# DaehwanKimLab/centrifuge

Hardware: NVIDIA H100
Metric: reads/sec (100 bp SE classification) (higher is better)
Workload: dtype u64

## Files before the change

### centrifuge_b200/capi.py

```python
import ctypes as C
import os

import numpy as np

HERE = os.path.dirname(os.path.abspath(__file__))
LIB_PATH = os.path.join(HERE, "libcfb200.so")

CFB_UID_NONE = 0xFFFFFFFF
REC_DTYPE = np.dtype([("taxid", "<u8"), ("score", "<u4"), ("hitlen", "<u4"), ("uid", "<u4"), ("pad", "<u4")])

_lib = None


class CfbError(RuntimeError):
    pass


class IndexInfo(C.Structure):
    _fields_ = [("len", C.c_uint64), ("num_sides", C.c_uint64), ("n_seqs", C.c_uint64), ("n_tax_nodes", C.c_uint64),
                ("n_boundaries", C.c_uint64), ("line_rate", C.c_int32), ("off_rate", C.c_int32), ("ftab_chars", C.c_int32),
                ("sample_bytes", C.c_int32), ("compressed", C.c_int32), ("device", C.c_int32), ("device_bytes", C.c_uint64)]


class IndexTables(C.Structure):
# ... 267 lines not shown
        out = np.zeros(3 * n, dtype=np.uint64)
        _ck(lib().cfb_counts_dense(self.h, C.c_int(1 if global_ else 0), _p(out, C.c_uint64), C.c_uint64(out.size)))
        return out.reshape(3, n)

    def comm_init_rank(self, nranks, rank, uid):
        buf = (C.c_uint8 * 128).from_buffer_copy(bytes(uid))
        _ck(lib().cfb_comm_init_rank(self.h, C.c_int(nranks), C.c_int(rank), buf))

    def counts_allreduce(self, out=None):
        arr = (C.c_void_p * 1)(self.h)
        _ck(lib().cfb_counts_allreduce(arr, C.c_int(1), _p(out, C.c_uint64) if out is not None else None, C.c_uint64(out.size if out is not None else 0)))

    def requests(self):
        out = (C.c_uint64 * 5)()
        _ck(lib().cfb_ctx_requests(self.h, out))
        return dict(zip(["rank16", "ftab2", "ftabk", "walk8", "ftabd"], [int(x) for x in out]))

    def request_breakdown(self):
        out = (C.c_uint64 * 8)()
        _ck(lib().cfb_ctx_request_breakdown(self.h, out))
        names = ["rank16_w1", "rank16_w2_4", "rank16_w5", "walk8_try_row", "walk8_ok_row", "walk8_try_range", "walk8_ok_range", "walk8_ok_w5"]
        return dict(zip(names, [int(x) for x in out]))

    def counters(self):
        out = (C.c_uint64 * 8)()
        _ck(lib().cfb_ctx_counters(self.h, out))
        names = ["units", "partial_searches", "ftab_probes", "sides_search", "walk_steps", "rows_resolved", "lf_steps", "ext_searches"]
        return dict(zip(names, [int(x) for x in out]))

    def launches(self):
        n = C.c_uint64()
        _ck(lib().cfb_ctx_kernel_launches(self.h, C.byref(n)))
        return int(n.value)

    def close(self):
        if self.h:
            lib().cfb_ctx_destroy(self.h)
            self.h = C.c_void_p()


def comm_unique_id():
    buf = (C.c_uint8 * 128)()
    _ck(lib().cfb_comm_unique_id(buf))
    return bytes(buf)


def comm_init_all(contexts):
    arr = (C.c_void_p * len(contexts))(*[c.h for c in contexts])
    _ck(lib().cfb_comm_init_all(arr, C.c_int(len(contexts))))


def counts_allreduce_all(contexts):
    arr = (C.c_void_p * len(contexts))(*[c.h for c in contexts])
    _ck(lib().cfb_counts_allreduce(arr, C.c_int(len(contexts)), None, C.c_uint64(0)))


def gather_ceiling(index, table, n_requests=1 << 30):
    g, ms = C.c_double(), C.c_double()
    _ck(lib().cfb_gather_ceiling(index.h, C.c_int(table), C.c_uint64(n_requests), C.byref(g), C.byref(ms)))
    return float(g.value), float(ms.value)


def test_lf(index, rows, chars):
    rows = np.ascontiguousarray(rows, dtype=np.uint64)
    chars = np.ascontiguousarray(chars, dtype=np.uint8)
    out = np.zeros(len(rows), dtype=np.uint64)
    _ck(lib().cfb_test_lf(index.h, _p(rows, C.c_uint64), _p(chars, C.c_uint8), C.c_uint64(len(rows)), _p(out, C.c_uint64)))
    return out


def test_resolve(index, rows):
    rows = np.ascontiguousarray(rows, dtype=np.uint64)
    out = np.zeros(len(rows), dtype=np.uint32)
    _ck(lib().cfb_test_resolve(index.h, _p(rows, C.c_uint64), C.c_uint64(len(rows)), _p(out, C.c_uint32)))
    return out


class BuildOpts(C.Structure):
    _fields_ = [("out_base", C.c_char_p), ("fasta", C.POINTER(C.c_char_p)), ("n_fasta", C.c_int32),
                ("synth_genera", C.c_uint32), ("synth_species", C.c_uint32), ("synth_len", C.c_uint64), ("synth_seed", C.c_uint64),
                ("synth_div", C.c_double), ("conversion_table", C.c_char_p), ("taxonomy_tree", C.c_char_p), ("name_table", C.c_char_p),
                ("size_table", C.c_char_p), ("ftab_chars", C.c_int32), ("off_rate", C.c_int32), ("device", C.c_int32), ("verbose", C.c_int32),
# ... 82 lines not shown
```

### centrifuge_b200/csrc/cf_logic.h

```cpp
#ifndef CF_LOGIC_H_
#define CF_LOGIC_H_

#include <stdint.h>

#ifdef __CUDACC__
#define CFB_HD __host__ __device__ __forceinline__
#define CFB_HDN __host__ __device__
#else
#define CFB_HD inline
#define CFB_HDN inline
#endif

namespace cfb {

static const uint64_t kOff = 0xffffffffffffffffull;
static const uint64_t kUnk = 0xfffffffffffffffeull;
static const uint32_t kBwNone = 0xffffffffu;

struct IndexView {
	const uint64_t* sides;
	const uint64_t* ftab;
	const uint64_t* eftab;
	const uint16_t* sample16;
	const uint32_t* sample32;
// ... 11 lines not shown
	const uint32_t* rtab32;
	const uint64_t* ftabk;
	const uint64_t* walk8;
	uint64_t walk8_rows;
	int32_t  ftabd_chars;
	uint64_t len, zoff, zside, fchr[4], last_boundary, num_sides;
	uint32_t zoffc, n_boundaries, n_seqs, n_host;
	int32_t  off_rate, ftab_chars, bshift, ftabk_chars;
};

struct Params {
	uint32_t khits, min_hitlen, ihits, increment;
	uint32_t tree_traverse, class_rank_slot;
};

struct HitRec { uint64_t top, bot; uint32_t bwoff, len; };

static const uint64_t kRowMask = (1ull << 40) - 1ull, kRowStart = 1ull << 63, kRowSameTs = 1ull << 58;

struct Counters {
	unsigned long long units, partial_searches, ftab_probes, sides_search, walk_steps, rows_resolved, lf_steps, ext_searches;
	unsigned long long req_rank16, req_ftab2, req_ftabk, req_walk8, req_ftabd;
	unsigned long long r16_w1, r16_w2_4, r16_w5, w8_try_row, w8_ok_row, w8_try_range, w8_ok_range, w8_ok_w5;
};

CFB_HD int popc64(uint64_t x) {
#ifdef __CUDA_ARCH__
	return __popcll(x);
#else
	return __builtin_popcountll(x);
#endif
}
CFB_HD uint32_t ctz32(uint32_t x) {
#ifdef __CUDA_ARCH__
	return (uint32_t)(__ffs(x) - 1);
#else
	return (uint32_t)__builtin_ctz(x);
#endif
}

static const uint64_t kOccMask = 0x7fffffffffffffffull;
CFB_HD uint64_t r16_entry(uint64_t row, int c) { return (row >> 6) * 4 + (uint64_t)c; }
CFB_HD uint64_t r16_lf(const IndexView& v, uint64_t row, int c, uint64_t occ, uint64_t bits) {
	return v.fchr[c] + (occ & kOccMask) + (uint64_t)popc64(bits & (((uint64_t)1 << (row & 63)) - 1));
}

// ... 534 lines not shown
```

### centrifuge_b200/csrc/cf_multi.cuh

```cuda
#include <dlfcn.h>
#include <nccl.h>

extern "C" int cfb_ctx_count_records(cfb_ctx* c, int on) {
	if(!c) return fail(CFB_EINVAL, "null ctx");
	CK(cudaSetDevice(c->ix->device));
	if(on) { int rc = counts_init(c); if(rc) return rc; }
	c->fold_records = on != 0;
	return CFB_OK;
}
extern "C" int cfb_counts_taxids(cfb_ctx* c, uint64_t* taxid, uint64_t cap, uint64_t* n) {
	if(!c || !n) return fail(CFB_EINVAL, "null argument");
	CK(cudaSetDevice(c->ix->device));
	int rc = counts_init(c); if(rc) return rc;
	*n = c->cnt.n;
	if(taxid) { if(cap < c->cnt.n) return fail(CFB_EINVAL, "cfb_counts_taxids: buffer too small"); memcpy(taxid, c->cnt.h_taxid.data(), (size_t)c->cnt.n * 8); }
	return CFB_OK;
}
extern "C" int cfb_counts_reset(cfb_ctx* c) {
	if(!c) return fail(CFB_EINVAL, "null ctx");
	CK(cudaSetDevice(c->ix->device));
	if(!c->cnt.ready) return CFB_OK;
	CK(cudaDeviceSynchronize());
	CK(cudaMemset(c->cnt.total.p, 0, 3ull * c->cnt.n * 8)); CK(cudaMemset(c->cnt.global.p, 0, 3ull * c->cnt.n * 8));
	c->cnt.reduced = false;
// ... 129 lines not shown
}
extern "C" int cfb_comm_info(const cfb_ctx* c, int* rank, int* size, int* nccl_version) {
	if(!c) return fail(CFB_EINVAL, "null ctx");
	if(rank) *rank = c->comm_rank; if(size) *size = c->comm ? c->comm_size : 1;
	if(nccl_version) { *nccl_version = 0; if(g_nccl.lib) g_nccl.GetVersion(nccl_version); }
	return CFB_OK;
}

extern "C" int cfb_ctx_requests(cfb_ctx* c, uint64_t out[5]) {
	if(!c || !out) return fail(CFB_EINVAL, "null argument");
	CK(cudaSetDevice(c->ix->device));
	Counters h; CK(cudaMemcpy(&h, c->d_ctr, sizeof h, cudaMemcpyDeviceToHost));
	out[0] = h.req_rank16; out[1] = h.req_ftab2; out[2] = h.req_ftabk; out[3] = h.req_walk8; out[4] = h.req_ftabd;
	return CFB_OK;
}
extern "C" int cfb_ctx_request_breakdown(cfb_ctx* c, uint64_t out[8]) {
	if(!c || !out) return fail(CFB_EINVAL, "null argument");
	CK(cudaSetDevice(c->ix->device));
	Counters h; CK(cudaMemcpy(&h, c->d_ctr, sizeof h, cudaMemcpyDeviceToHost));
	out[0] = h.r16_w1; out[1] = h.r16_w2_4; out[2] = h.r16_w5;
	out[3] = h.w8_try_row; out[4] = h.w8_ok_row; out[5] = h.w8_try_range; out[6] = h.w8_ok_range; out[7] = h.w8_ok_w5;
	return CFB_OK;
}

__device__ __forceinline__ uint64_t gmix(uint64_t x) { x += 0x9E3779B97F4A7C15ull; x = (x ^ (x >> 30)) * 0xBF58476D1CE4E5B9ull; x = (x ^ (x >> 27)) * 0x94D049BB133111EBull; return x ^ (x >> 31); }
template <int W, int ILP>
__global__ void __launch_bounds__(128) k_gather_probe(const unsigned long long* __restrict__ a, uint64_t n, uint32_t iters, unsigned long long* sink) {
	const uint64_t tid = (uint64_t)blockIdx.x * blockDim.x + threadIdx.x;
	uint64_t h = gmix(tid * 0x2545F4914F6CDD1Dull + 1), acc = 0;
	for(uint32_t it = 0; it < iters; it++) {
		unsigned long long v[ILP][W];
		#pragma unroll
		for(int k = 0; k < ILP; k++) {
			h = gmix(h + k);
			const uint64_t u = h % n;
			if(W == 2) { const ulonglong2 q = __ldg(reinterpret_cast<const ulonglong2*>(a) + u); v[k][0] = q.x; v[k][W - 1] = q.y; }
			else v[k][0] = __ldg(a + u);
		}
		#pragma unroll
		for(int k = 0; k < ILP; k++) acc += W == 2 ? (v[k][0] ^ (v[k][W - 1] << 1)) : v[k][0];
	}
	if(acc == 0x123456789abcull) *sink = acc;
}
extern "C" int cfb_gather_ceiling(const cfb_index* ix, int table, uint64_t n_requests, double* g_requests_per_s, double* ms_out) {
	if(!ix || !g_requests_per_s || ix->device < 0) return fail(CFB_EINVAL, "cfb_gather_ceiling: bad argument");
	CK(cudaSetDevice(ix->device));
	const cfb_index_tables& t = ix->tables; const IndexView& v = ix->view;
	const unsigned long long* base = nullptr; uint64_t n = 0; int W = 1;
	switch(table) {
		case 0: base = (const unsigned long long*)v.rank16; n = t.rank16_bytes / 16; W = 2; break;
		case 1: base = (const unsigned long long*)v.ftabk; n = t.ftabk_bytes / 16; W = 2; break;
		case 2: base = (const unsigned long long*)v.walk8; n = t.walk8_bytes / 8; W = 1; break;
		case 3: base = v.rtab32 ? (const unsigned long long*)v.rtab32 : (const unsigned long long*)v.rtab16; n = t.resolve_table_bytes / 8; W = 1; break;
		case 4: break;
		default: return fail(CFB_EINVAL, "cfb_gather_ceiling: unknown table %d", table);
	}
	if(!base || n == 0) return fail(CFB_EINVAL, "cfb_gather_ceiling: table %d is not built", table);
	const int ILP = 4, threads = 128;
	const int blocks = ix->sm_count * 16;
	const uint64_t per_iter = (uint64_t)blocks * threads * ILP;
	const uint32_t iters = (uint32_t)std::max<uint64_t>(1, n_requests / per_iter);
	unsigned long long* sink = nullptr; CK(cudaMalloc((void**)&sink, 8));
	cudaEvent_t e0, e1; CK(cudaEventCreate(&e0)); CK(cudaEventCreate(&e1));
	auto launch = [&](uint32_t it) {
		if(W == 2) k_gather_probe<2, 4><<<blocks, threads>>>(base, n, it, sink); else k_gather_probe<1, 4><<<blocks, threads>>>(base, n, it, sink);
	};
	launch(std::max<uint32_t>(1, iters / 16)); CK(cudaDeviceSynchronize());
	CK(cudaEventRecord(e0)); launch(iters); CK(cudaEventRecord(e1)); CK(cudaEventSynchronize(e1));
	float ms = 0; CK(cudaEventElapsedTime(&ms, e0, e1));
	cudaEventDestroy(e0); cudaEventDestroy(e1); cudaFree(sink);
	CK(cudaGetLastError());
	*g_requests_per_s = (double)per_iter * iters / ((double)ms * 1e6);
	if(ms_out) *ms_out = ms;
	return CFB_OK;
}
```

### centrifuge_b200/csrc/cfb200.cu

```cuda
#include "../../include/cfb200.h"
#include "cf_index.h"
#include "cf_kernels.cuh"

#include <algorithm>
#include <atomic>
#include <mutex>
#include <thread>
#include <fcntl.h>
#include <unistd.h>
#include <cstdarg>
#include <cstdio>
#include <cstring>
#include <set>
#include <string>
#include <vector>

using namespace cfb;

enum { M_DONE = 0, M_FTAB = 1, M_LF = 2, M_NEED = 3, M_FTABK = 4 };

struct SearchArgs {
	IndexView v; Params p; BatchView b;
	HitRec* hits; uint32_t* nhits; uint32_t cap;
	unsigned long long* task_ctr64; uint32_t ntasks, chunk;
	unsigned int* overflow;
	Counters* ctr;
	const uint64_t* pk; const uint32_t* nm; uint32_t W;
	uint32_t keep_short;
};

__device__ __forceinline__ uint64_t shl64(uint64_t v, uint32_t n) {
	uint64_t r; asm("shl.b64 %0, %1, %2;" : "=l"(r) : "l"(v), "r"(n)); return r;
}
__device__ __forceinline__ uint64_t shr64(uint64_t v, uint32_t n) {
	uint64_t r; asm("shr.b64 %0, %1, %2;" : "=l"(r) : "l"(v), "r"(n)); return r;
}

struct PackArgs { BatchView b; uint64_t* pk; uint32_t* nm; uint32_t W; };

__device__ __forceinline__ uint32_t load4(const uint8_t* base, uint64_t off) {
	const uint32_t* w = reinterpret_cast<const uint32_t*>(base + (off & ~3ull));
	return __funnelshift_r(w[0], w[1], (uint32_t)(off & 3) * 8);
// ... 18 lines not shown
		const uint64_t lo = strand ? off + k * 32 : off + (len - k * 32 - cnt);
		#pragma unroll
		for(uint32_t g = 0; g < 32; g += 4) {
			if(g < cnt) {
				const uint32_t keep = cnt - g >= 4 ? 0xffffffffu : ((1u << (8 * (cnt - g))) - 1u);
				const uint32_t v = load4(a.b.bases, lo + g) & keep;
				const uint32_t nb = __vcmpne4(v & 0xFCFCFCFCu, 0u) & 0x01010101u;
				uint32_t b2 = v & 0x03030303u;
				if(strand) b2 ^= 0x03030303u & keep;
				b2 &= ~(nb * 3u);
				w |= (uint64_t)squeeze4x2(b2) << (2 * g);
				n |= squeeze4x1(nb) << g;
			}
		}
		if(!strand) {
			uint64_t x = __brevll(w);
			x = ((x >> 1) & 0x5555555555555555ull) | ((x & 0x5555555555555555ull) << 1);
			w = x >> (2 * (32 - cnt)); n = __brev(n) >> (32 - cnt);
		}
	}
	a.pk[i] = w; a.nm[i] = n;
}

struct WarpPool { unsigned long long base, end; };
__device__ __forceinline__ bool pool_take(WarpPool& P, bool want, unsigned long long* ctr, unsigned long long total, unsigned chunk, unsigned long long& out) {
	const unsigned need = __ballot_sync(0xffffffffu, want);
	if(!need) return false;
	const unsigned lane = threadIdx.x & 31;
	const unsigned cnt = __popc(need), r = __popc(need & ((1u << lane) - 1u));
	const unsigned long long avail = P.end - P.base;
	unsigned long long nb = 0;
	const bool refill = avail < cnt;
	if(refill) { if(lane == 0) nb = atomicAdd(ctr, (unsigned long long)chunk); nb = __shfl_sync(0xffffffffu, nb, 0); }
	unsigned long long t, lim;
	if(r < avail) { t = P.base + r; lim = P.end; }
	else { t = nb + (r - avail); lim = nb + chunk < total ? nb + chunk : total; }
	if(refill) { P.base = nb + (cnt - avail); P.end = nb + chunk < total ? nb + chunk : total; if(P.base > P.end) P.base = P.end; }
	else P.base += cnt;
	out = t;
	return want && t < lim;
}

__device__ __forceinline__ uint64_t even_bits(uint64_t x) {
	x &= 0x5555555555555555ull;
	x = (x | (x >> 1)) & 0x3333333333333333ull;
	x = (x | (x >> 2)) & 0x0f0f0f0f0f0f0f0full;
	x = (x | (x >> 4)) & 0x00ff00ff00ff00ffull;
	x = (x | (x >> 8)) & 0x0000ffff0000ffffull;
	x = (x | (x >> 16)) & 0x00000000ffffffffull;
	return x;
}

__global__ void k_build_rank16(const uint64_t* sides, uint64_t num_sides, uint64_t zside, uint32_t zoffc, uint64_t* r16) {
	const uint64_t b = (uint64_t)blockIdx.x * blockDim.x + threadIdx.x;
	if(b > num_sides * 6) return;
	const bool sentinel = b == num_sides * 6;
// ... 67 lines not shown
	uint64_t y = ~0ull;
	if(death) {
		uint8_t dv[64];
		uint64_t t1[4], b1[4]; lf4(v, r16, top, bot, t1, b1);
		for(int c0 = 0; c0 < 4; c0++) {
			if(b1[c0] <= t1[c0]) { for(int r = 0; r < 16; r++) dv[c0 | (r << 2)] = 1; continue; }
			uint64_t t2[4], b2[4]; lf4(v, r16, t1[c0], b1[c0], t2, b2);
			for(int c1 = 0; c1 < 4; c1++) {
				if(b2[c1] <= t2[c1]) { for(int c2 = 0; c2 < 4; c2++) dv[c0 | (c1 << 2) | (c2 << 4)] = 2; continue; }
				uint64_t t3[4], b3[4]; lf4(v, r16, t2[c1], b2[c1], t3, b3);
				for(int c2 = 0; c2 < 4; c2++) dv[c0 | (c1 << 2) | (c2 << 4)] = b3[c2] <= t3[c2] ? 3 : 0;
			}
		}
		y = 0;
		for(int e = 0; e < 64; e++) if(dv[e] == 0) y |= 1ull << e;
		for(uint32_t e = 0; e < 64; e++) if(ftabk_death(y, e) != dv[e]) { y = ~0ull; break; }
	}
	const uint64_t w = bot - top;
	out[fk] = make_ulonglong2(top | ((w < kFtabkWide ? w : kFtabkWide) << 40), y);
}

template <int RW> struct ReadRegs {
	uint64_t rw[RW]; uint32_t nw[RW];
	__device__ __forceinline__ void load(const uint64_t* pk, const uint32_t* nm, uint32_t W) {
		#pragma unroll
		for(int k = 0; k < RW; k++) { rw[k] = (uint32_t)k < W ? __ldg(pk + k) : 0ull; nw[k] = (uint32_t)k < W ? __ldg(nm + k) : 0u; }
	}
	__device__ __forceinline__ uint64_t word(uint32_t k) const {
		uint64_t v = 0;
		#pragma unroll
		for(int q = 0; q < RW; q++) if((uint32_t)q == k) v = rw[q];
		return v;
	}
	__device__ __forceinline__ uint32_t nword(uint32_t k) const {
		uint32_t v = 0;
		#pragma unroll
		for(int q = 0; q < RW; q++) if((uint32_t)q == k) v = nw[q];
		return v;
	}
	__device__ __forceinline__ int base(uint32_t p) const {
		const uint32_t k = p >> 5, sh = p & 31;
		return ((nword(k) >> sh) & 1u) ? 4 : (int)((word(k) >> (2 * sh)) & 3);
	}
	__device__ __forceinline__ void window(uint32_t p, uint64_t& win, uint32_t& nwin) const {
		const uint32_t k = p >> 5, sh = p & 31;
		win = shr64(word(k), 2 * sh) | shl64(word(k + 1), 64 - 2 * sh);
		nwin = (uint32_t)(((uint64_t)nword(k) | ((uint64_t)nword(k + 1) << 32)) >> sh);
	}
};

template <bool REQS, int RW>
__global__ void __launch_bounds__(kSearchThreads, !REQS && RW <= 5 ? 8 : 1) k_search_t(const SearchArgs a) {
	const ulonglong2* r16 = reinterpret_cast<const ulonglong2*>(a.v.rank16);
	const ulonglong2* ftab2 = reinterpret_cast<const ulonglong2*>(a.v.ftab2);
	const ulonglong2* ftabk = reinterpret_cast<const ulonglong2*>(a.v.ftabk);
	const uint32_t fk = a.v.ftabk ? (uint32_t)a.v.ftabk_chars : 0u;
	const uint32_t fc = (uint32_t)a.v.ftab_chars;
	const unsigned long long* w8 = reinterpret_cast<const unsigned long long*>(a.v.walk8);
	const uint32_t fd = (fk == 0 || a.p.min_hitlen < (uint32_t)a.v.ftabd_chars) ? 0u : (uint32_t)a.v.ftabd_chars;
	ReadRegs<RW> rd;
	uint64_t top = 0, bot = 0, fi = 0;
	uint32_t rlen = 0, tid = 0, cur = 0, dep = 0, offset = 0, nh = 0, nt = 0, slow_until = 0, fail_at = 0xffffffffu;
	bool nolong = true;
	int mode = M_NEED;
	unsigned long long q_r16 = 0, q_f2 = 0, q_fk = 0, q_w8 = 0;
	unsigned long long q_w1 = 0, q_w24 = 0, q_w5 = 0, j_row = 0, j_row_ok = 0, j_rng = 0, j_rng_ok = 0, j_w5_ok = 0;
	WarpPool pool; pool.base = pool.end = 0;
	bool more = true;

	auto emit = [&](uint64_t t, uint64_t b, uint32_t off, uint32_t len) {
		if(a.keep_short || len >= kLongLen) {
			if(nh < a.cap) { HitRec* h = a.hits + (size_t)tid * a.cap + nh; h->top = t; h->bot = b; h->bwoff = off; h->len = len; }
			else atomicExch(a.overflow, 1u);
			nh++;
		}
		nt++;
		if(len >= a.p.min_hitlen) nolong = false;
	};
	auto after_hit = [&](uint32_t hlen) -> bool {
		bool done = cur >= rlen;
		if(!done) { if(hlen > a.p.increment) cur += 1; if(cur + a.p.min_hitlen >= rlen) done = true; }
		if(done) { a.nhits[tid] = nh_pack(nh, nt, nolong); mode = M_NEED; return false; }
		return true;
	};
	auto start_search = [&]() {
		for(;;) {
			offset = cur;
			if(rlen - cur < fc) { emit(kOff, kOff, offset, rlen - offset); a.nhits[tid] = nh_pack(nh, nt, nolong); mode = M_NEED; return; }
			uint64_t win; uint32_t nwin; rd.window(cur, win, nwin);
			const uint32_t nbits = nwin & ((1u << fc) - 1u);
			if(nbits) {
				const uint32_t hl = (uint32_t)__ffs(nbits);
				cur += hl;
				emit(kOff, kOff, offset, hl);
				if(after_hit(hl)) continue; else return;
			}
			if(fk && rlen - cur >= fk && !(nwin & ((1u << fk) - 1u))) {
				fi = win & ((1ull << (2 * fk)) - 1ull);
				if(fd && rlen - cur >= fd && !(nwin & ((1u << fd) - 1u))) fi |= (64ull | ((win >> (2 * fk)) & 63ull)) << (2 * fk);
				mode = M_FTABK;
				return;
			}
			fi = win & ((1ull << (2 * fc)) - 1ull);
			mode = M_FTAB;
			return;
		}
	};
	auto hit_and_restart = [&]() {
		const uint32_t hl = dep - offset;
		emit(top, bot, offset, hl);
		cur = dep;
		if(after_hit(hl)) start_search();
	};

	for(;;) {
		{
			const bool want = mode == M_NEED;
			if(more) {
				unsigned long long t = 0;
				const bool got = pool_take(pool, want, a.task_ctr64, (unsigned long long)a.ntasks, a.chunk, t);
				if(want) {
					if(got) {
						tid = (uint32_t)t;
						const uint32_t per = 2u * (uint32_t)a.b.n_mates;
						const uint32_t unit = tid / per, rem = tid - unit * per;
						const int mate = (int)(rem >> 1);
						const uint8_t fl = a.b.flags ? a.b.flags[unit] : 3;
						nh = 0; nt = 0; rlen = a.b.len[mate][unit];
						if(!((fl >> mate) & 1) || rlen == 0) a.nhits[tid] = 0;
						else { rd.load(a.pk + (size_t)tid * a.W, a.nm + (size_t)tid * a.W, a.W); cur = 0; slow_until = 0; fail_at = 0xffffffffu; nolong = true; start_search(); }
					} else mode = M_DONE;
				}
				if(__any_sync(0xffffffffu, want && !got)) more = false;
			} else if(want) mode = M_DONE;
		}
		if(!__any_sync(0xffffffffu, mode != M_DONE)) break;
		int c = 4;
		const bool lf = mode == M_LF;
		bool range = false, jump = false, known_fail = false;
		const void* p0 = nullptr; const void* p1 = nullptr; uint32_t sub = 0;
		if(mode == M_FTAB) { p0 = ftab2 + fi; if(REQS) q_f2++; }
		else if(mode == M_FTABK) { p0 = ftabk + (fi & ((1ull << (2 * fk)) - 1ull)); if(REQS) q_fk++; }
		else if(lf) {
			c = rd.base(dep);
			if(c <= 3) {
				range = (bot - top) != 1;
				const uint64_t width = bot - top;
				if(dep == fail_at && !range) known_fail = true;
				else if(w8 && dep >= slow_until && rlen - dep >= 8 && bot <= a.v.walk8_rows) {
					jump = true; p0 = w8 + (top & ~1ull); sub = (uint32_t)(top & 1);
					if(range) { const uint64_t last = bot - 1; sub |= (uint32_t)(last & 1) << 1; if((last & ~1ull) != (top & ~1ull)) p1 = w8 + (last & ~1ull); }
					if(REQS) { q_w8 += p1 ? 2 : 1; if(range) j_rng++; else j_row++; }
				} else {
					p0 = r16 + r16_entry(top, c);
					if(range && (bot >> 6) != (top >> 6)) p1 = r16 + r16_entry(bot, c);
					if(REQS) { const uint32_t n = p1 ? 2 : 1; q_r16 += n; if(width == 1) q_w1 += n; else if(width <= 4) q_w24 += n; else q_w5 += n; }
				}
			}
		}
		ulonglong2 e = make_ulonglong2(0, 0), bq;
		asm volatile("{\n\t.reg .pred p;\n\tsetp.ne.u64 p, %2, 0;\n\t@p ld.global.nc.v2.u64 {%0, %1}, [%2];\n\t}" : "+l"(e.x), "+l"(e.y) : "l"(p0));
		bq = e;
		asm volatile("{\n\t.reg .pred p;\n\tsetp.ne.u64 p, %2, 0;\n\t@p ld.global.nc.v2.u64 {%0, %1}, [%2];\n\t}" : "+l"(bq.x), "+l"(bq.y) : "l"(p1));
		const ulonglong2 tq = e;
		if(mode == M_FTABK) {
			const uint32_t ext = (uint32_t)(fi >> (2 * fk));
			const uint32_t dv = ext ? ftabk_death(e.y, ext & 63u) : 0u;
			const uint64_t width = e.x >> 40;
			if(dv) {
				const uint32_t hl = fk + dv - 1u;
				emit(kUnk, kUnk, offset, hl);
				cur += hl;
				if(after_hit(hl)) start_search();
			} else if(width != 0 && width != kFtabkWide) {
				top = e.x & kRowMask; bot = top + width; dep = cur + fk;
				if(dep < rlen) mode = M_LF; else hit_and_restart();
			} else { fi &= (1ull << (2 * fc)) - 1ull; mode = M_FTAB; }
		} else if(mode == M_FTAB) {
			top = e.x; bot = e.y;
			dep = cur + fc;
			if(bot <= top) {
				const uint32_t hl = dep - offset;
				emit(kOff, kOff, offset, hl);
				cur = dep;
				if(after_hit(hl)) start_search();
			} else if(dep < rlen) mode = M_LF;
			else hit_and_restart();
		} else if(jump) {
			uint64_t win; uint32_t nwin; rd.window(dep, win, nwin);
			const uint64_t w = (sub & 1u) ? e.y : e.x;
			const uint64_t wl = range ? ((sub & 2u) ? bq.y : bq.x) : w;
			const uint32_t st = walk8_steps(w, win, nwin), sb = range ? walk8_steps(wl, win, nwin) : st;
			if((st & sb) == 8u) {
				if(REQS) { if(range) j_rng_ok++; else j_row_ok++; if(bot - top >= 5) j_w5_ok++; }
				top = w & kWalkRowMask; bot = (wl & kWalkRowMask) + 1; dep += 8;
				if(dep >= rlen) hit_and_restart();
			} else {
				slow_until = dep + walk8_retry(st, sb);
				if(!range) fail_at = dep + st;
			}
		} else if(lf) {
			bool fail = c > 3 || known_fail;
			uint64_t t = 0, b = 0;
			if(!fail) {
				t = r16_lf(a.v, top, c, tq.x, tq.y);
				if(range) b = r16_lf(a.v, bot, c, bq.x, bq.y);
				else {
					if(!((tq.y >> (top & 63)) & 1ull)) fail = true;
					b = t + 1;
				}
				if(b <= t) fail = true;
			}
			if(fail) hit_and_restart();
			else { top = t; bot = b; dep++; if(dep >= rlen) hit_and_restart(); }
		}
	}
	if(REQS && a.ctr) {
		atomicAdd(&a.ctr->req_rank16, q_r16); atomicAdd(&a.ctr->req_ftab2, q_f2); atomicAdd(&a.ctr->req_ftabk, q_fk); atomicAdd(&a.ctr->req_walk8, q_w8);
		atomicAdd(&a.ctr->r16_w1, q_w1); atomicAdd(&a.ctr->r16_w2_4, q_w24); atomicAdd(&a.ctr->r16_w5, q_w5);
		atomicAdd(&a.ctr->w8_try_row, j_row); atomicAdd(&a.ctr->w8_ok_row, j_row_ok); atomicAdd(&a.ctr->w8_try_range, j_rng); atomicAdd(&a.ctr->w8_ok_range, j_rng_ok); atomicAdd(&a.ctr->w8_ok_w5, j_w5_ok);
	}
}

struct UnitArgs {
	IndexView v; Params p; BatchView b;
	HitRec* hits; uint32_t* nhits; uint32_t cap;
	uint32_t* nrows;
	uint64_t* row_off;
	unsigned long long* row_total;
	uint64_t* rows; uint32_t* ids; uint64_t rows_cap;
	Entry* entries; TaxCnt* tcs; OutRec* recs_sparse; uint32_t* nout;
	unsigned int* overflow;
	Counters* ctr;
	HitRec* regen; uint32_t* regen_n; unsigned long long* regen_ctr; uint64_t regen_slots; uint32_t full_cap; uint32_t keep_short;
};

__device__ uint32_t search_strand_dev(const IndexView& v, const Params& p, const uint8_t* fw, uint32_t len, int strand, HitRec* hits, uint32_t cap) {
	const ulonglong2* r16 = reinterpret_cast<const ulonglong2*>(v.rank16);
	const ulonglong2* ftab2 = reinterpret_cast<const ulonglong2*>(v.ftab2);
	const ulonglong2* ftabk = reinterpret_cast<const ulonglong2*>(v.ftabk);
	const uint32_t fc = (uint32_t)v.ftab_chars, fk = v.ftabk ? (uint32_t)v.ftabk_chars : 0u;
	auto base = [&](uint32_t d) -> int { return seq_at(fw, len, strand, len - 1 - d); };
	uint32_t cur = 0, n = 0;
// ... 278 lines not shown

enum { R_DONE = 0, R_WALK = 1, R_SAMPLE = 2, R_NEED = 3 };
struct ResolveArgs {
	IndexView v; const uint64_t* rows; uint32_t* ids; uint16_t* ids16; const uint64_t* total; uint64_t rows_cap;
	unsigned long long* task_ctr; uint32_t chunk; Counters* ctr;
};
__device__ __forceinline__ int group_lf(const IndexView& v, uint64_t row, const ulonglong2 e, uint64_t& next) {
	const unsigned gl = threadIdx.x & 3, gbase = threadIdx.x & 28, gmask = 0xFu << gbase;
	const uint64_t mine = r16_lf(v, row, (int)gl, e.x, e.y);
	const int src = __ffs((__ballot_sync(gmask, (e.y >> (row & 63)) & 1ull) >> gbase) & 0xFu) - 1;
	next = __shfl_sync(gmask, mine, gbase + (src < 0 ? 0 : src));
	return src;
}

template <bool COUNT, bool IDENT>
__global__ void __launch_bounds__(kSearchThreads) k_resolve_c(const ResolveArgs a) {
	const unsigned lane = threadIdx.x & 31, gl = lane & 3, gbase = lane & 28, gmask = 0xFu << gbase;
	const ulonglong2* r16 = reinterpret_cast<const ulonglong2*>(a.v.rank16);
	uint64_t n = *a.total; if(n > a.rows_cap) return;
	const uint64_t lowmask = ((uint64_t)1 << a.v.off_rate) - 1;
	uint64_t idx = 0, row = 0;
	int mode = R_NEED;
	unsigned long long c_walk = 0, c_rows = 0;
	WarpPool pool; pool.base = pool.end = 0;
	bool more = true;
	auto put = [&](uint32_t v) { if(IDENT && a.ids16) a.ids16[idx] = (uint16_t)v; else a.ids[idx] = v; };
	auto settle = [&](uint64_t r) -> int {
		if(r == a.v.zoff) { if(gl == 0) put(0); return R_NEED; }
		if((r & lowmask) == 0) return R_SAMPLE;
		return R_WALK;
	};
	for(;;) {
		{
			const bool want = mode == R_NEED;
			if(more) {
				unsigned long long t = 0;
				bool got = pool_take(pool, want && gl == 0, a.task_ctr, (unsigned long long)n, a.chunk, t);
				t = __shfl_sync(0xffffffffu, t, gbase); got = __shfl_sync(0xffffffffu, (int)got, gbase) != 0;
				if(want) {
					if(got) { idx = t; row = IDENT ? idx : (a.rows[idx] & kRowMask); if(COUNT && gl == 0) c_rows++; mode = settle(row); }
					else mode = R_DONE;
				}
				if(__any_sync(0xffffffffu, want && !got)) more = false;
			} else if(want) mode = R_DONE;
		}
		if(!__any_sync(0xffffffffu, mode != R_DONE)) break;
		ulonglong2 e = make_ulonglong2(0, 0); uint32_t samp = 0;
// ... 928 lines not shown
```

### include/cfb200.h

```cpp
#ifndef CFB200_H_
#define CFB200_H_

#include <stddef.h>
#include <stdint.h>

#ifdef __cplusplus
extern "C" {
#endif

#define CFB_OK        0
#define CFB_EINVAL   -1
#define CFB_EIO      -2
#define CFB_ENOMEM   -3
#define CFB_ENODEV   -4
#define CFB_ECUDA    -5
#define CFB_EFORMAT  -6

#define CFB_UID_NONE 0xFFFFFFFFu

typedef struct cfb_index cfb_index;
typedef struct cfb_ctx   cfb_ctx;

int cfb_index_load(const char* basename, int device, cfb_index** out);
#define CFB_LOAD_NO_RESOLVE_TABLE 1u
// ... 107 lines not shown
	const uint64_t* multi; uint64_t n_multi; uint32_t multi_stride;
} cfb_text_result;
int cfb_text_submit(cfb_ctx*, int slot, const void* text_a, uint64_t bytes_a, const void* text_b, uint64_t bytes_b,
                    uint64_t n_records, const cfb_text_opts*);
int cfb_text_wait(cfb_ctx*, int slot, int discard, cfb_text_result* out);
int cfb_ctx_set_columns(cfb_ctx*, const char* cols);
int cfb_text_species(cfb_ctx*, uint64_t* taxid, uint64_t* n_reads, uint64_t* n_unique, uint64_t* n_obs1, uint64_t cap, uint64_t* n);

int cfb_ctx_count_records(cfb_ctx*, int on);
int cfb_counts_taxids(cfb_ctx*, uint64_t* taxid, uint64_t cap, uint64_t* n);
int cfb_counts_reset(cfb_ctx*);
int cfb_counts_read(cfb_ctx*, int global, uint64_t* taxid, uint64_t* n_reads, uint64_t* n_unique, uint64_t* n_obs1, uint64_t cap, uint64_t* n);
int cfb_counts_dense(cfb_ctx*, int global, uint64_t* out, uint64_t cap);
#define CFB_COMM_ID_BYTES 128
int cfb_comm_unique_id(uint8_t id[CFB_COMM_ID_BYTES]);
int cfb_comm_init_rank(cfb_ctx*, int nranks, int rank, const uint8_t id[CFB_COMM_ID_BYTES]);
int cfb_comm_init_all(cfb_ctx* const* ctxs, int n);
int cfb_comm_info(const cfb_ctx*, int* rank, int* size, int* nccl_version);
int cfb_counts_allreduce(cfb_ctx* const* ctxs, int n, uint64_t* dense_out, uint64_t cap);

int cfb_ctx_requests(cfb_ctx*, uint64_t out[5]);
int cfb_ctx_request_breakdown(cfb_ctx*, uint64_t out[8]);
int cfb_gather_ceiling(const cfb_index*, int table, uint64_t n_requests, double* g_requests_per_s, double* ms);

int cfb_ctx_counters(cfb_ctx*, uint64_t out[8]);
int cfb_ctx_kernel_launches(const cfb_ctx*, uint64_t* n);

int   cfb_device_count(void);
void* cfb_host_alloc(size_t bytes);
void  cfb_host_free(void*);

int cfb_test_lf(const cfb_index*, const uint64_t* rows, const uint8_t* chars, uint64_t n, uint64_t* out);
int cfb_test_resolve(const cfb_index*, const uint64_t* rows, uint64_t n, uint32_t* out);
int cfb_test_parse(const char* path, int fasta, int trim5, int trim3, uint32_t seed, const char* out_path);
int cfb_test_host_path(const char* index_base, const char* reads_a, const char* reads_b, int fasta, int khits, uint32_t seed,
                       int trim5, int trim3, const uint32_t* rec_off, const cfb_rec* recs, uint64_t n_units,
                       const char* out_tsv, const char* out_report, const char* out_kreport);

const char* cfb_last_error(void);
const char* cfb_version(void);

typedef struct {
	const char* out_base;
	const char* const* fasta; int32_t n_fasta;
	uint32_t synth_genera, synth_species; uint64_t synth_len, synth_seed; double synth_div;
	const char* conversion_table;
// ... 33 lines not shown
```

Before: 282.0 million.

## Restructure search loop to fold task loads into batched predicated gathers and prefetch pool

The search kernel no longer loads a new read's packed words, length and flags inside the pool-take branch. It adds an M_TASK mode so those loads are issued as predicated non-coherent loads alongside the iteration's index-table gathers, letting their latencies overlap. The emit/restart lambdas are replaced by a single inline restart loop. The work pool also prefetches the next chunk's atomicAdd ahead of need. The change adds per-iteration clock and path instrumentation behind the REQS template and a configurable gather-rate probe, at the cost of one extra loop trip per new read and more registers.

```diff
diff --git a/centrifuge_b200/capi.py b/centrifuge_b200/capi.py
--- a/centrifuge_b200/capi.py
+++ b/centrifuge_b200/capi.py
@@ -313,6 +313,12 @@
         names = ["rank16_w1", "rank16_w2_4", "rank16_w5", "walk8_try_row", "walk8_ok_row", "walk8_try_range", "walk8_ok_range", "walk8_ok_w5"]
         return dict(zip(names, [int(x) for x in out]))
 
+    def search_iter_stats(self):
+        out = (C.c_uint64 * 8)()
+        _ck(lib().cfb_ctx_search_iter_stats(self.h, out))
+        names = ["warp_iters", "lane_requests", "consumer_paths", "restart_paths", "task_iters", "clk_head", "clk_wait", "clk_tail"]
+        return dict(zip(names, [int(x) for x in out]))
+
     def counters(self):
         out = (C.c_uint64 * 8)()
         _ck(lib().cfb_ctx_counters(self.h, out))
@@ -349,6 +355,12 @@
 def gather_ceiling(index, table, n_requests=1 << 30):
     g, ms = C.c_double(), C.c_double()
     _ck(lib().cfb_gather_ceiling(index.h, C.c_int(table), C.c_uint64(n_requests), C.byref(g), C.byref(ms)))
+    return float(g.value), float(ms.value)
+
+
+def gather_rate(index, table, n_requests, ctas_per_sm, ilp):
+    g, ms = C.c_double(), C.c_double()
+    _ck(lib().cfb_gather_rate(index.h, C.c_int(table), C.c_uint64(n_requests), C.c_int(ctas_per_sm), C.c_int(ilp), C.byref(g), C.byref(ms)))
     return float(g.value), float(ms.value)
 
 
diff --git a/centrifuge_b200/csrc/cf_logic.h b/centrifuge_b200/csrc/cf_logic.h
--- a/centrifuge_b200/csrc/cf_logic.h
+++ b/centrifuge_b200/csrc/cf_logic.h
@@ -57,6 +57,7 @@
 	unsigned long long units, partial_searches, ftab_probes, sides_search, walk_steps, rows_resolved, lf_steps, ext_searches;
 	unsigned long long req_rank16, req_ftab2, req_ftabk, req_walk8, req_ftabd;
 	unsigned long long r16_w1, r16_w2_4, r16_w5, w8_try_row, w8_ok_row, w8_try_range, w8_ok_range, w8_ok_w5;
+	unsigned long long it_warp, it_lane_req, it_consumers, it_restarts, it_task, clk_head, clk_wait, clk_tail;
 };
 
 CFB_HD int popc64(uint64_t x) {
diff --git a/centrifuge_b200/csrc/cf_multi.cuh b/centrifuge_b200/csrc/cf_multi.cuh
--- a/centrifuge_b200/csrc/cf_multi.cuh
+++ b/centrifuge_b200/csrc/cf_multi.cuh
@@ -175,6 +175,14 @@
 	out[3] = h.w8_try_row; out[4] = h.w8_ok_row; out[5] = h.w8_try_range; out[6] = h.w8_ok_range; out[7] = h.w8_ok_w5;
 	return CFB_OK;
 }
+extern "C" int cfb_ctx_search_iter_stats(cfb_ctx* c, uint64_t out[8]) {
+	if(!c || !out) return fail(CFB_EINVAL, "null argument");
+	CK(cudaSetDevice(c->ix->device));
+	Counters h; CK(cudaMemcpy(&h, c->d_ctr, sizeof h, cudaMemcpyDeviceToHost));
+	out[0] = h.it_warp; out[1] = h.it_lane_req; out[2] = h.it_consumers; out[3] = h.it_restarts; out[4] = h.it_task;
+	out[5] = h.clk_head; out[6] = h.clk_wait; out[7] = h.clk_tail;
+	return CFB_OK;
+}
 
 __device__ __forceinline__ uint64_t gmix(uint64_t x) { x += 0x9E3779B97F4A7C15ull; x = (x ^ (x >> 30)) * 0xBF58476D1CE4E5B9ull; x = (x ^ (x >> 27)) * 0x94D049BB133111EBull; return x ^ (x >> 31); }
 template <int W, int ILP>
@@ -195,8 +203,8 @@
 	}
 	if(acc == 0x123456789abcull) *sink = acc;
 }
-extern "C" int cfb_gather_ceiling(const cfb_index* ix, int table, uint64_t n_requests, double* g_requests_per_s, double* ms_out) {
-	if(!ix || !g_requests_per_s || ix->device < 0) return fail(CFB_EINVAL, "cfb_gather_ceiling: bad argument");
+extern "C" int cfb_gather_rate(const cfb_index* ix, int table, uint64_t n_requests, int ctas_per_sm, int ilp, double* g_requests_per_s, double* ms_out) {
+	if(!ix || !g_requests_per_s || ix->device < 0 || ctas_per_sm < 1 || (ilp != 1 && ilp != 2 && ilp != 4)) return fail(CFB_EINVAL, "cfb_gather_rate: bad argument");
 	CK(cudaSetDevice(ix->device));
 	const cfb_index_tables& t = ix->tables; const IndexView& v = ix->view;
 	const unsigned long long* base = nullptr; uint64_t n = 0; int W = 1;
@@ -206,17 +214,18 @@
 		case 2: base = (const unsigned long long*)v.walk8; n = t.walk8_bytes / 8; W = 1; break;
 		case 3: base = v.rtab32 ? (const unsigned long long*)v.rtab32 : (const unsigned long long*)v.rtab16; n = t.resolve_table_bytes / 8; W = 1; break;
 		case 4: break;
-		default: return fail(CFB_EINVAL, "cfb_gather_ceiling: unknown table %d", table);
-	}
-	if(!base || n == 0) return fail(CFB_EINVAL, "cfb_gather_ceiling: table %d is not built", table);
-	const int ILP = 4, threads = 128;
-	const int blocks = ix->sm_count * 16;
-	const uint64_t per_iter = (uint64_t)blocks * threads * ILP;
+		default: return fail(CFB_EINVAL, "cfb_gather_rate: unknown table %d", table);
+	}
+	if(!base || n == 0) return fail(CFB_EINVAL, "cfb_gather_rate: table %d is not built", table);
+	const int threads = 128;
+	const int blocks = ix->sm_count * ctas_per_sm;
+	const uint64_t per_iter = (uint64_t)blocks * threads * ilp;
 	const uint32_t iters = (uint32_t)std::max<uint64_t>(1, n_requests / per_iter);
 	unsigned long long* sink = nullptr; CK(cudaMalloc((void**)&sink, 8));
 	cudaEvent_t e0, e1; CK(cudaEventCreate(&e0)); CK(cudaEventCreate(&e1));
 	auto launch = [&](uint32_t it) {
-		if(W == 2) k_gather_probe<2, 4><<<blocks, threads>>>(base, n, it, sink); else k_gather_probe<1, 4><<<blocks, threads>>>(base, n, it, sink);
+		if(W == 2) { if(ilp == 4) k_gather_probe<2, 4><<<blocks, threads>>>(base, n, it, sink); else if(ilp == 2) k_gather_probe<2, 2><<<blocks, threads>>>(base, n, it, sink); else k_gather_probe<2, 1><<<blocks, threads>>>(base, n, it, sink); }
+		else { if(ilp == 4) k_gather_probe<1, 4><<<blocks, threads>>>(base, n, it, sink); else if(ilp == 2) k_gather_probe<1, 2><<<blocks, threads>>>(base, n, it, sink); else k_gather_probe<1, 1><<<blocks, threads>>>(base, n, it, sink); }
 	};
 	launch(std::max<uint32_t>(1, iters / 16)); CK(cudaDeviceSynchronize());
 	CK(cudaEventRecord(e0)); launch(iters); CK(cudaEventRecord(e1)); CK(cudaEventSynchronize(e1));
@@ -227,3 +236,6 @@
 	if(ms_out) *ms_out = ms;
 	return CFB_OK;
 }
+extern "C" int cfb_gather_ceiling(const cfb_index* ix, int table, uint64_t n_requests, double* g_requests_per_s, double* ms_out) {
+	return cfb_gather_rate(ix, table, n_requests, 16, 4, g_requests_per_s, ms_out);
+}
diff --git a/centrifuge_b200/csrc/cfb200.cu b/centrifuge_b200/csrc/cfb200.cu
--- a/centrifuge_b200/csrc/cfb200.cu
+++ b/centrifuge_b200/csrc/cfb200.cu
@@ -17,7 +17,7 @@
 
 using namespace cfb;
 
-enum { M_DONE = 0, M_FTAB = 1, M_LF = 2, M_NEED = 3, M_FTABK = 4 };
+enum { M_DONE = 0, M_FTAB = 1, M_LF = 2, M_NEED = 3, M_FTABK = 4, M_TASK = 5 };
 
 struct SearchArgs {
 	IndexView v; Params p; BatchView b;
@@ -82,7 +82,10 @@
 	a.pk[i] = w; a.nm[i] = n;
 }
 
-struct WarpPool { unsigned long long base, end; };
+struct WarpPool { unsigned long long base = 0, end = 0, next = 0; bool ahead = false; };
+__device__ __forceinline__ void pool_ahead(WarpPool& P, unsigned long long* ctr, unsigned chunk) {
+	if(!P.ahead && P.end - P.base < 32) { if((threadIdx.x & 31) == 0) P.next = atomicAdd(ctr, (unsigned long long)chunk); P.ahead = true; }
+}
 __device__ __forceinline__ bool pool_take(WarpPool& P, bool want, unsigned long long* ctr, unsigned long long total, unsigned chunk, unsigned long long& out) {
 	const unsigned need = __ballot_sync(0xffffffffu, want);
 	if(!need) return false;
@@ -91,7 +94,7 @@
 	const unsigned long long avail = P.end - P.base;
 	unsigned long long nb = 0;
 	const bool refill = avail < cnt;
-	if(refill) { if(lane == 0) nb = atomicAdd(ctr, (unsigned long long)chunk); nb = __shfl_sync(0xffffffffu, nb, 0); }
+	if(refill) { if(lane == 0) nb = P.ahead ? P.next : atomicAdd(ctr, (unsigned long long)chunk); nb = __shfl_sync(0xffffffffu, nb, 0); P.ahead = false; }
 	unsigned long long t, lim;
 	if(r < avail) { t = P.base + r; lim = P.end; }
 	else { t = nb + (r - avail); lim = nb + chunk < total ? nb + chunk : total; }
@@ -205,10 +208,6 @@
 
 template <int RW> struct ReadRegs {
 	uint64_t rw[RW]; uint32_t nw[RW];
-	__device__ __forceinline__ void load(const uint64_t* pk, const uint32_t* nm, uint32_t W) {
-		#pragma unroll
-		for(int k = 0; k < RW; k++) { rw[k] = (uint32_t)k < W ? __ldg(pk + k) : 0ull; nw[k] = (uint32_t)k < W ? __ldg(nm + k) : 0u; }
-	}
 	__device__ __forceinline__ uint64_t word(uint32_t k) const {
 		uint64_t v = 0;
 		#pragma unroll
@@ -231,6 +230,19 @@
 		nwin = (uint32_t)(((uint64_t)nword(k) | ((uint64_t)nword(k + 1) << 32)) >> sh);
 	}
 };
+
+__device__ __forceinline__ void ld_if(ulonglong2& v, const void* p) {
+	asm volatile("{\n\t.reg .pred p;\n\tsetp.ne.u64 p, %2, 0;\n\t@p ld.global.nc.v2.u64 {%0, %1}, [%2];\n\t}" : "+l"(v.x), "+l"(v.y) : "l"(p));
+}
+__device__ __forceinline__ void ld_if(uint64_t& v, const uint64_t* p, bool on) {
+	asm volatile("{\n\t.reg .pred p;\n\tsetp.ne.u32 p, %2, 0;\n\t@p ld.global.nc.u64 %0, [%1];\n\t}" : "+l"(v) : "l"(p), "r"((uint32_t)on));
+}
+__device__ __forceinline__ void ld_if(uint32_t& v, const uint32_t* p, bool on) {
+	asm volatile("{\n\t.reg .pred p;\n\tsetp.ne.u32 p, %2, 0;\n\t@p ld.global.nc.u32 %0, [%1];\n\t}" : "+r"(v) : "l"(p), "r"((uint32_t)on));
+}
+__device__ __forceinline__ void ld_if(uint32_t& v, const uint8_t* p, bool on) {
+	asm volatile("{\n\t.reg .pred p;\n\tsetp.ne.u32 p, %2, 0;\n\t@p ld.global.nc.u8 %0, [%1];\n\t}" : "+r"(v) : "l"(p), "r"((uint32_t)on));
+}
 
 template <bool REQS, int RW>
 __global__ void __launch_bounds__(kSearchThreads, !REQS && RW <= 5 ? 8 : 1) k_search_t(const SearchArgs a) {
@@ -241,85 +253,39 @@
 	const uint32_t fc = (uint32_t)a.v.ftab_chars;
 	const unsigned long long* w8 = reinterpret_cast<const unsigned long long*>(a.v.walk8);
 	const uint32_t fd = (fk == 0 || a.p.min_hitlen < (uint32_t)a.v.ftabd_chars) ? 0u : (uint32_t)a.v.ftabd_chars;
+	const uint32_t msh = a.b.n_mates == 2 ? 2u : 1u;
 	ReadRegs<RW> rd;
+	#pragma unroll
+	for(int k = 0; k < RW; k++) { rd.rw[k] = 0; rd.nw[k] = 0; }
 	uint64_t top = 0, bot = 0, fi = 0;
 	uint32_t rlen = 0, tid = 0, cur = 0, dep = 0, offset = 0, nh = 0, nt = 0, slow_until = 0, fail_at = 0xffffffffu;
 	bool nolong = true;
 	int mode = M_NEED;
 	unsigned long long q_r16 = 0, q_f2 = 0, q_fk = 0, q_w8 = 0;
 	unsigned long long q_w1 = 0, q_w24 = 0, q_w5 = 0, j_row = 0, j_row_ok = 0, j_rng = 0, j_rng_ok = 0, j_w5_ok = 0;
-	WarpPool pool; pool.base = pool.end = 0;
+	unsigned long long s_trips = 0, s_lreq = 0, s_cons = 0, s_rest = 0, s_task = 0, s_head = 0, s_wait = 0, s_tail = 0;
+	uint32_t paths = 0; long long t_top = 0, t_issue = 0, t_data = 0;
+	WarpPool pool;
 	bool more = true;
 
-	auto emit = [&](uint64_t t, uint64_t b, uint32_t off, uint32_t len) {
-		if(a.keep_short || len >= kLongLen) {
-			if(nh < a.cap) { HitRec* h = a.hits + (size_t)tid * a.cap + nh; h->top = t; h->bot = b; h->bwoff = off; h->len = len; }
-			else atomicExch(a.overflow, 1u);
-			nh++;
-		}
-		nt++;
-		if(len >= a.p.min_hitlen) nolong = false;
-	};
-	auto after_hit = [&](uint32_t hlen) -> bool {
-		bool done = cur >= rlen;
-		if(!done) { if(hlen > a.p.increment) cur += 1; if(cur + a.p.min_hitlen >= rlen) done = true; }
-		if(done) { a.nhits[tid] = nh_pack(nh, nt, nolong); mode = M_NEED; return false; }
-		return true;
-	};
-	auto start_search = [&]() {
-		for(;;) {
-			offset = cur;
-			if(rlen - cur < fc) { emit(kOff, kOff, offset, rlen - offset); a.nhits[tid] = nh_pack(nh, nt, nolong); mode = M_NEED; return; }
-			uint64_t win; uint32_t nwin; rd.window(cur, win, nwin);
-			const uint32_t nbits = nwin & ((1u << fc) - 1u);
-			if(nbits) {
-				const uint32_t hl = (uint32_t)__ffs(nbits);
-				cur += hl;
-				emit(kOff, kOff, offset, hl);
-				if(after_hit(hl)) continue; else return;
-			}
-			if(fk && rlen - cur >= fk && !(nwin & ((1u << fk) - 1u))) {
-				fi = win & ((1ull << (2 * fk)) - 1ull);
-				if(fd && rlen - cur >= fd && !(nwin & ((1u << fd) - 1u))) fi |= (64ull | ((win >> (2 * fk)) & 63ull)) << (2 * fk);
-				mode = M_FTABK;
-				return;
-			}
-			fi = win & ((1ull << (2 * fc)) - 1ull);
-			mode = M_FTAB;
-			return;
-		}
-	};
-	auto hit_and_restart = [&]() {
-		const uint32_t hl = dep - offset;
-		emit(top, bot, offset, hl);
-		cur = dep;
-		if(after_hit(hl)) start_search();
-	};
-
 	for(;;) {
+		if(REQS) { paths = 0; t_top = clock64(); }
 		{
 			const bool want = mode == M_NEED;
 			if(more) {
 				unsigned long long t = 0;
 				const bool got = pool_take(pool, want, a.task_ctr64, (unsigned long long)a.ntasks, a.chunk, t);
 				if(want) {
-					if(got) {
-						tid = (uint32_t)t;
-						const uint32_t per = 2u * (uint32_t)a.b.n_mates;
-						const uint32_t unit = tid / per, rem = tid - unit * per;
-						const int mate = (int)(rem >> 1);
-						const uint8_t fl = a.b.flags ? a.b.flags[unit] : 3;
-						nh = 0; nt = 0; rlen = a.b.len[mate][unit];
-						if(!((fl >> mate) & 1) || rlen == 0) a.nhits[tid] = 0;
-						else { rd.load(a.pk + (size_t)tid * a.W, a.nm + (size_t)tid * a.W, a.W); cur = 0; slow_until = 0; fail_at = 0xffffffffu; nolong = true; start_search(); }
-					} else mode = M_DONE;
+					if(got) { tid = (uint32_t)t; mode = M_TASK; if(REQS) paths |= 1u << 17; }
+					else mode = M_DONE;
 				}
 				if(__any_sync(0xffffffffu, want && !got)) more = false;
+				else pool_ahead(pool, a.task_ctr64, a.chunk);
 			} else if(want) mode = M_DONE;
 		}
 		if(!__any_sync(0xffffffffu, mode != M_DONE)) break;
 		int c = 4;
-		const bool lf = mode == M_LF;
+		const bool lf = mode == M_LF, task = mode == M_TASK;
 		bool range = false, jump = false, known_fail = false;
 		const void* p0 = nullptr; const void* p1 = nullptr; uint32_t sub = 0;
 		if(mode == M_FTAB) { p0 = ftab2 + fi; if(REQS) q_f2++; }
@@ -341,35 +307,52 @@
 				}
 			}
 		}
-		ulonglong2 e = make_ulonglong2(0, 0), bq;
-		asm volatile("{\n\t.reg .pred p;\n\tsetp.ne.u64 p, %2, 0;\n\t@p ld.global.nc.v2.u64 {%0, %1}, [%2];\n\t}" : "+l"(e.x), "+l"(e.y) : "l"(p0));
-		bq = e;
-		asm volatile("{\n\t.reg .pred p;\n\tsetp.ne.u64 p, %2, 0;\n\t@p ld.global.nc.v2.u64 {%0, %1}, [%2];\n\t}" : "+l"(bq.x), "+l"(bq.y) : "l"(p1));
-		const ulonglong2 tq = e;
-		if(mode == M_FTABK) {
+		const uint32_t unit = tid >> msh, mate = (tid >> 1) & (msh - 1u);
+		const uint64_t* tpk = a.pk + (size_t)tid * a.W; const uint32_t* tnm = a.nm + (size_t)tid * a.W;
+		uint32_t fl = 3;
+		if(REQS) { if(p0) s_lreq++; t_issue = clock64(); }
+		const bool two = p1 != nullptr;
+		ulonglong2 e = make_ulonglong2(0, 0), e2 = make_ulonglong2(0, 0);
+		ld_if(e, p0);
+		ld_if(e2, p1);
+		ld_if(rlen, (mate ? a.b.len[1] : a.b.len[0]) + unit, task);
+		ld_if(fl, a.b.flags + unit, task && a.b.flags != nullptr);
+		#pragma unroll
+		for(int k = 0; k < RW; k++) { ld_if(rd.rw[k], tpk + k, task && (uint32_t)k < a.W); ld_if(rd.nw[k], tnm + k, task && (uint32_t)k < a.W); }
+		if(REQS) {
+			if(__any_sync(0xffffffffu, (e.x ^ e2.y ^ rd.rw[RW - 1] ^ rd.nw[RW - 1] ^ rlen ^ fl) == 0x9e3779b97f4a7c15ull)) s_task += 1ull << 40;
+			t_data = clock64();
+		}
+		const ulonglong2 tq = e, bq = two ? e2 : e;
+		bool ended = false, stop = false, fresh = false;
+		uint64_t h_top = kOff, h_bot = kOff; uint32_t hl = 0;
+		if(task) {
+			if(REQS) paths |= 1u;
+			#pragma unroll
+			for(int k = 0; k < RW; k++) if((uint32_t)k >= a.W) { rd.rw[k] = 0; rd.nw[k] = 0; }
+			nh = 0; nt = 0;
+			if(!((fl >> mate) & 1) || rlen == 0) { a.nhits[tid] = 0; mode = M_NEED; }
+			else { cur = 0; slow_until = 0; fail_at = 0xffffffffu; nolong = true; fresh = true; }
+		} else if(mode == M_FTABK) {
+			if(REQS) paths |= 2u;
 			const uint32_t ext = (uint32_t)(fi >> (2 * fk));
 			const uint32_t dv = ext ? ftabk_death(e.y, ext & 63u) : 0u;
 			const uint64_t width = e.x >> 40;
 			if(dv) {
-				const uint32_t hl = fk + dv - 1u;
-				emit(kUnk, kUnk, offset, hl);
-				cur += hl;
-				if(after_hit(hl)) start_search();
+				hl = fk + dv - 1u; h_top = h_bot = kUnk; cur += hl; ended = true;
 			} else if(width != 0 && width != kFtabkWide) {
 				top = e.x & kRowMask; bot = top + width; dep = cur + fk;
-				if(dep < rlen) mode = M_LF; else hit_and_restart();
+				if(dep < rlen) mode = M_LF; else stop = true;
 			} else { fi &= (1ull << (2 * fc)) - 1ull; mode = M_FTAB; }
 		} else if(mode == M_FTAB) {
+			if(REQS) paths |= 4u;
 			top = e.x; bot = e.y;
 			dep = cur + fc;
-			if(bot <= top) {
-				const uint32_t hl = dep - offset;
-				emit(kOff, kOff, offset, hl);
-				cur = dep;
-				if(after_hit(hl)) start_search();
-			} else if(dep < rlen) mode = M_LF;
-			else hit_and_restart();
+			if(bot <= top) { hl = dep - offset; cur = dep; ended = true; }
+			else if(dep < rlen) mode = M_LF;
+			else stop = true;
 		} else if(jump) {
+			if(REQS) paths |= 8u;
 			uint64_t win; uint32_t nwin; rd.window(dep, win, nwin);
 			const uint64_t w = (sub & 1u) ? e.y : e.x;
 			const uint64_t wl = range ? ((sub & 2u) ? bq.y : bq.x) : w;
@@ -377,12 +360,13 @@
 			if((st & sb) == 8u) {
 				if(REQS) { if(range) j_rng_ok++; else j_row_ok++; if(bot - top >= 5) j_w5_ok++; }
 				top = w & kWalkRowMask; bot = (wl & kWalkRowMask) + 1; dep += 8;
-				if(dep >= rlen) hit_and_restart();
+				stop = dep >= rlen;
 			} else {
 				slow_until = dep + walk8_retry(st, sb);
 				if(!range) fail_at = dep + st;
 			}
 		} else if(lf) {
+			if(REQS) paths |= 16u;
 			bool fail = c > 3 || known_fail;
 			uint64_t t = 0, b = 0;
 			if(!fail) {
@@ -394,14 +378,57 @@
 				}
 				if(b <= t) fail = true;
 			}
-			if(fail) hit_and_restart();
-			else { top = t; bot = b; dep++; if(dep >= rlen) hit_and_restart(); }
+			if(fail) stop = true;
+			else { top = t; bot = b; dep++; stop = dep >= rlen; }
+		}
+		if(stop) { h_top = top; h_bot = bot; hl = dep - offset; cur = dep; ended = true; }
+		#pragma unroll 1
+		while(ended || fresh) {
+			if(ended) {
+				if(REQS) paths |= 1u << 16;
+				if(a.keep_short || hl >= kLongLen) {
+					if(nh < a.cap) { HitRec* h = a.hits + (size_t)tid * a.cap + nh; h->top = h_top; h->bot = h_bot; h->bwoff = offset; h->len = hl; }
+					else atomicExch(a.overflow, 1u);
+					nh++;
+				}
+				nt++;
+				if(hl >= a.p.min_hitlen) nolong = false;
+				ended = false;
+				bool done = cur >= rlen;
+				if(!done) { if(hl > a.p.increment) cur += 1; if(cur + a.p.min_hitlen >= rlen) done = true; }
+				if(done) { a.nhits[tid] = nh_pack(nh, nt, nolong); mode = M_NEED; break; }
+			}
+			if(REQS) paths |= 1u << 18;
+			fresh = false;
+			offset = cur; h_top = h_bot = kOff;
+			if(rlen - cur < fc) { hl = rlen - cur; cur = rlen; ended = true; continue; }
+			uint64_t win; uint32_t nwin; rd.window(cur, win, nwin);
+			const uint32_t nbits = nwin & ((1u << fc) - 1u);
+			if(nbits) { hl = (uint32_t)__ffs(nbits); cur += hl; ended = true; continue; }
+			if(fk && rlen - cur >= fk && !(nwin & ((1u << fk) - 1u))) {
+				fi = win & ((1ull << (2 * fk)) - 1ull);
+				if(fd && rlen - cur >= fd && !(nwin & ((1u << fd) - 1u))) fi |= (64ull | ((win >> (2 * fk)) & 63ull)) << (2 * fk);
+				mode = M_FTABK;
+			} else {
+				fi = win & ((1ull << (2 * fc)) - 1ull);
+				mode = M_FTAB;
+			}
+		}
+		if(REQS) {
+			const uint32_t all = __reduce_or_sync(0xffffffffu, paths);
+			s_trips++; s_cons += __popc(all & 0xffffu); s_rest += __popc(all >> 16); if(all & (1u << 17)) s_task++;
+			const long long t_end = clock64(); s_head += t_issue - t_top; s_wait += t_data - t_issue; s_tail += t_end - t_data;
 		}
 	}
 	if(REQS && a.ctr) {
 		atomicAdd(&a.ctr->req_rank16, q_r16); atomicAdd(&a.ctr->req_ftab2, q_f2); atomicAdd(&a.ctr->req_ftabk, q_fk); atomicAdd(&a.ctr->req_walk8, q_w8);
 		atomicAdd(&a.ctr->r16_w1, q_w1); atomicAdd(&a.ctr->r16_w2_4, q_w24); atomicAdd(&a.ctr->r16_w5, q_w5);
 		atomicAdd(&a.ctr->w8_try_row, j_row); atomicAdd(&a.ctr->w8_ok_row, j_row_ok); atomicAdd(&a.ctr->w8_try_range, j_rng); atomicAdd(&a.ctr->w8_ok_range, j_rng_ok); atomicAdd(&a.ctr->w8_ok_w5, j_w5_ok);
+		atomicAdd(&a.ctr->it_lane_req, s_lreq);
+		if((threadIdx.x & 31) == 0) {
+			atomicAdd(&a.ctr->it_warp, s_trips); atomicAdd(&a.ctr->it_consumers, s_cons); atomicAdd(&a.ctr->it_restarts, s_rest); atomicAdd(&a.ctr->it_task, s_task & ((1ull << 40) - 1ull));
+			atomicAdd(&a.ctr->clk_head, s_head); atomicAdd(&a.ctr->clk_wait, s_wait); atomicAdd(&a.ctr->clk_tail, s_tail);
+		}
 	}
 }
 
@@ -726,7 +753,7 @@
 	uint64_t idx = 0, row = 0;
 	int mode = R_NEED;
 	unsigned long long c_walk = 0, c_rows = 0;
-	WarpPool pool; pool.base = pool.end = 0;
+	WarpPool pool;
 	bool more = true;
 	auto put = [&](uint32_t v) { if(IDENT && a.ids16) a.ids16[idx] = (uint16_t)v; else a.ids[idx] = v; };
 	auto settle = [&](uint64_t r) -> int {
diff --git a/include/cfb200.h b/include/cfb200.h
--- a/include/cfb200.h
+++ b/include/cfb200.h
@@ -153,6 +153,8 @@
 int cfb_ctx_requests(cfb_ctx*, uint64_t out[5]);
 int cfb_ctx_request_breakdown(cfb_ctx*, uint64_t out[8]);
 int cfb_gather_ceiling(const cfb_index*, int table, uint64_t n_requests, double* g_requests_per_s, double* ms);
+int cfb_gather_rate(const cfb_index*, int table, uint64_t n_requests, int ctas_per_sm, int ilp, double* g_requests_per_s, double* ms);
+int cfb_ctx_search_iter_stats(cfb_ctx*, uint64_t out[8]);
 
 int cfb_ctx_counters(cfb_ctx*, uint64_t out[8]);
 int cfb_ctx_kernel_launches(const cfb_ctx*, uint64_t* n);
```

Result: faster. 292.5 million, median of 6 (+3.7%).
